# DataZooDE/anofox-forecast

Hardware: AMD Instinct MI355X
Metric: series/sec fit+forecast, AutoETS h=28 on M5-shape batches (higher is better)
Workload: dtype f64

## Files before the change

### anofox-forecast_amd/csrc/det_math.hpp

```cpp
#pragma once
#include <hip/hip_runtime.h>
#include <stdint.h>

namespace anofox {

__device__ __forceinline__ double dm_from_bits(uint64_t u) { return __longlong_as_double((long long)u); }
__device__ __forceinline__ uint64_t dm_bits(double x) { return (uint64_t)__double_as_longlong(x); }

__device__ __forceinline__ double dm_log(double x)
{
    const double ln2_hi = 6.93147180369123816490e-01, ln2_lo = 1.90821492927058770002e-10;
    const double Lg1 = 6.666666666666735130e-01, Lg2 = 3.999999999940941908e-01,
                 Lg3 = 2.857142874366239149e-01, Lg4 = 2.222219843214978396e-01,
                 Lg5 = 1.818357216161805012e-01, Lg6 = 1.531383769920937332e-01,
                 Lg7 = 1.479819860511658591e-01;
    uint64_t u = dm_bits(x);
    uint32_t hx = (uint32_t)(u >> 32);
    int k = 0;
    if (x != x) return x;
    if (hx < 0x00100000u || (hx >> 31)) {
        if ((u << 1) == 0) return -__builtin_huge_val();
        if (hx >> 31) return __builtin_nan("");
        k -= 54;
        x *= 18014398509481984.0;
// ... 145 lines not shown
    const double r2 = r * r;
    const double pa = fma(r, 1.0 / 3.0, -0.5);
    const double pb = fma(r, 0.2, -0.25);
    const double pl = fma(r2, fma(r2, -1.0 / 6.0, pb), pa);
    const double l1p = fma(r2, pl, r);
    const double de = (double)e;
    const double lg = fma(de, ln2_hi, ic.y) + fma(de, ln2_lo, l1p);
    const double t = y * lg;
    const double dn = __builtin_rint(n_per_ln2 * t);
    const double s = fma(-dn, L_lo, fma(-dn, L_hi, t));
    const double s2 = s * s;
    const double qa = fma(s, 1.0 / 6.0, 0.5);
    const double qb = fma(s, 1.0 / 120.0, 1.0 / 24.0);
    const double q = fma(s2, fma(s2, 1.0 / 720.0, qb), qa);
    const double p = fma(s2, q, s);
    const int n = (int)dn;
    const double tv = tab[DM_POW_R64 * (n & 63) + cp.o64];
    const double ev = fma(tv, p, tv);
    return __builtin_ldexp(ev, n >> 6);
}

constexpr int DM_POW_NEAR1_DEG = 11;
constexpr double DM_POW_NEAR1_R = 0x1p-4;
struct DmPowNear1 { double c[DM_POW_NEAR1_DEG + 1]; };
__device__ __forceinline__ void dm_pow_near1_coef(double y, DmPowNear1 &o)
{
    constexpr double inv[DM_POW_NEAR1_DEG + 1] = { 0.0, 1.0, 1.0 / 2.0, 1.0 / 3.0, 1.0 / 4.0, 1.0 / 5.0, 1.0 / 6.0, 1.0 / 7.0,
                                                   1.0 / 8.0, 1.0 / 9.0, 1.0 / 10.0, 1.0 / 11.0 };
    o.c[0] = 1.0;
    o.c[1] = y;
#pragma unroll
    for (int k = 2; k <= DM_POW_NEAR1_DEG; k++) o.c[k] = o.c[k - 1] * ((y - (double)(k - 1)) * inv[k]);
}
__device__ __forceinline__ double dm_pow_near1(double r, const DmPowNear1 &o)
{
    double p = o.c[DM_POW_NEAR1_DEG];
#pragma unroll
    for (int k = DM_POW_NEAR1_DEG - 1; k >= 1; k--) p = fma(p, r, o.c[k]);
    return fma(p, r, 1.0);
}

__device__ __forceinline__ double dm_recip(double d)
{
    const double x0 = __builtin_amdgcn_rcp(d);
    const double e0 = fma(-d, x0, 1.0);
    const double x1 = fma(x0, e0, x0);
    const double e1 = fma(-d, x1, 1.0);
    const double x2 = fma(x1, e1, x1);
    const double e2 = fma(-d, x2, 1.0);
    return fma(e2, x2, x2);
}
__device__ __forceinline__ bool dm_recip_ok(double d) { const double a = fabs(d); return a >= 0x1p-1000 && a <= 0x1p+1000; }

__device__ __forceinline__ double dm_pow_pos(double x, double y) { return dm_exp(y * dm_log(x)); }

}
```

### anofox-forecast_amd/csrc/ets_device.hpp

```cpp
#pragma once
#include <hip/hip_runtime.h>
#include <type_traits>
#include "det_math.hpp"
#include "nm.hpp"

namespace anofox {

enum { C_NONE = 0, C_ADD = 1, C_MUL = 2 };

constexpr double ETS_TOL = 1.0e-10;
constexpr double ETS_HUGEN = 1.0e10;
constexpr double ETS_LN2 = 0.693147180559945309417232121458;
constexpr double PAR_LO = 1.0e-4, PAR_HI = 0.9999, PHI_LO = 0.8, PHI_HI = 0.98;
constexpr int ETS_MERGED_LDS_PERIOD = 16;
constexpr int ETS_LDS_PERIOD = 64;
constexpr int ETS_MAX_PERIOD = 2048;

struct SeriesView {
    const double *y;
    size_t ld;
    int len;
    int wave_len;
    int wave_min_len;
    int rows;
// ... 52 lines not shown
    static constexpr bool CLASSIC = false;
};

struct EtsPar { double alpha, bstar, phi, beta, gamma; DmPowLane pl; DmPowNear1 pc; };
struct EtsState { double l, b, sse, mant; int eacc; int bad; double f; double dlo, dhi, bmin; double rfar; };

template <class Cfg>
__device__ __forceinline__ void ets_unpack(const double (&x)[Cfg::DIM], EtsPar &p)
{
    int k = 0;
    p.alpha = x[k++];
    p.bstar = 0.0;
    double gstar = 0.0;
    p.phi = 1.0;
    if constexpr (Cfg::T != C_NONE) p.bstar = x[k++];
    if constexpr (Cfg::S != C_NONE) gstar = x[k++];
    if constexpr (Cfg::D) p.phi = x[k++];
    p.beta = p.alpha * p.bstar;
    p.gamma = gstar * (1.0 - p.alpha);
}

template <class Cfg, bool NEAR = false>
__device__ __forceinline__ void ets_step(const EtsPar &p, EtsState &st, double y, double &s)
{
    if constexpr (Cfg::ADDITIVE) {
        double phib = 0.0, q = st.l;
        if constexpr (Cfg::T == C_ADD) {
            phib = Cfg::D ? p.phi * st.b : st.b;
            q = st.l + phib;
        }
        double f = q;
        if constexpr (Cfg::S == C_ADD) f = q + s;
        double e = y - f;
        st.sse = fma(e, e, st.sse);
        st.l = fma(p.alpha, e, q);
        st.f = f;
        if constexpr (Cfg::T == C_ADD) st.b = fma(p.beta, e, phib);
        if constexpr (Cfg::S == C_ADD) s = fma(p.gamma, e, s);
    } else {
        double phib = 0.0, q = st.l;
        if constexpr (Cfg::T == C_ADD) {
            phib = Cfg::D ? p.phi * st.b : st.b;
            q = st.l + phib;
        } else if constexpr (Cfg::T == C_MUL) {
            if constexpr (Cfg::D) {
                const double r = st.b - 1.0;
                phib = dm_pow_near1(r, p.pc);
                if constexpr (NEAR) st.rfar = __builtin_fmax(st.rfar, fabs(r));
                else if (!(fabs(r) <= DM_POW_NEAR1_R)) {
                    if (!(st.b >= 0x1p-1000 && st.b <= 0x1p+1000)) st.bad = 1;
                    phib = dm_pow_step(st.b, p.phi, p.pl);
                }
            } else {
                st.bmin = __builtin_fmin(st.bmin, st.b);
                phib = st.b;
            }
            q = st.l * phib;
        }
        double f = q;
        if constexpr (Cfg::S == C_ADD) f = q + s;
        else if constexpr (Cfg::S == C_MUL) f = q * s;
        st.f = f;
        auto recip = [&](const double d) __attribute__((always_inline)) {
            const double ad = fabs(d);
            st.dlo = __builtin_fmin(st.dlo, ad);
            st.dhi = __builtin_fmax(st.dhi, ad);
            return dm_recip(d);
        };
        if constexpr (Cfg::E == C_MUL) {
            static_assert(Cfg::S != C_ADD, "multiplicative error with an additive season is not a valid spec");
            const double rf = recip(f);
            const double eps = (y - f) * rf;
            st.mant = st.mant * fabs(f);
            st.sse = fma(eps, eps, st.sse);
            const double qe = q * eps;
            st.l = fma(p.alpha, qe, q);
            if constexpr (Cfg::T == C_ADD) st.b = fma(p.beta, qe, phib);
            else if constexpr (Cfg::T == C_MUL) st.b = fma(p.beta, phib * eps, phib);
            if constexpr (Cfg::S == C_MUL) s = fma(p.gamma, s * eps, s);
        } else {
            const double e = y - f;
            st.sse = fma(e, e, st.sse);
            if constexpr (Cfg::S == C_MUL && Cfg::T == C_MUL) {
                const double R = recip(f * st.l);
                const double esl = e * (R * q);
                const double es = esl * st.l;
                const double sl = s * st.l;
                st.l = fma(p.alpha, es, q);
                st.b = fma(p.beta, esl, phib);
                s = fma(p.gamma, e * (R * sl), s);
            } else if constexpr (Cfg::S == C_MUL) {
                const double R = recip(f);
                const double es = e * (R * q);
                st.l = fma(p.alpha, es, q);
                if constexpr (Cfg::T == C_ADD) st.b = fma(p.beta, es, phib);
                s = fma(p.gamma, e * (R * s), s);
            } else {
                static_assert(Cfg::T == C_MUL, "general class: a multiplicative component");
                const double rl = recip(st.l);
                st.l = fma(p.alpha, e, q);
                st.b = fma(p.beta, e * rl, phib);
                if constexpr (Cfg::S == C_ADD) s = fma(p.gamma, e, s);
            }
        }
    }
}

template <class Cfg>
__device__ __forceinline__ void ets_renorm(EtsState &st)
{
    if constexpr (Cfg::E == C_MUL) {
        int ex;
        st.mant = frexp(st.mant, &ex);
        st.eacc += ex;
    }
}

template <class Cfg>
__device__ __forceinline__ double ets_objective_value(const EtsState &st, int n)
// ... 10 lines not shown
    if (lik < -1.0e10) lik = -1.0e10;
    return lik;
}

struct EtsInit {
    double l0, b0;
    const double *fig;
    size_t fig_ld;
    int m;
};

struct EtsFinalOut {
    double *yhat; int h; double *sse_out;
    double *fitted; size_t fitted_ld; double *states; size_t states_ld;
    double mean; double *var_out;
};

template <class Cfg, int MS, int K, bool FINAL, class YT = double>
__device__ __forceinline__ void ets_pass(const SeriesView &v, const EtsInit &in,
                                         const double (&cand)[K][Cfg::DIM], double (&fout)[K],
                                         double *ring, const EtsFinalOut *fin)
{
    static_assert((Cfg::S == C_NONE) == (MS == 0), "MS == 0 iff no seasonal component");
    const int lane = threadIdx.x & (NM_BLOCK - 1);
    EtsPar par[K];
    EtsState st[K];
#pragma unroll
    for (int k = 0; k < K; k++) {
        ets_unpack<Cfg>(cand[k], par[k]);
        if constexpr (Cfg::T == C_MUL && Cfg::D) { par[k].pl = dm_pow_lane(); dm_pow_near1_coef(par[k].phi, par[k].pc); }
        st[k].l = in.l0; st[k].b = in.b0; st[k].sse = 0.0; st[k].mant = 1.0; st[k].eacc = 0; st[k].bad = 0;
        st[k].f = 0.0; st[k].dlo = __builtin_huge_val(); st[k].dhi = 0.0; st[k].bmin = __builtin_huge_val(); st[k].rfar = 0.0;

    }
    const double *yp = v.yb;
    const unsigned col_bytes = (unsigned)v.col * (unsigned)sizeof(YT);
    const size_t ld = v.ld;

    const int wave_len = __builtin_amdgcn_readfirstlane(v.wave_len);
    const int wave_min_len = __builtin_amdgcn_readfirstlane(v.wave_min_len);
    const int row_max = __builtin_amdgcn_readfirstlane(v.rows) - 1;
    constexpr int S_WIDE = std::is_same_v<YT, double> ? 1 : (Cfg::ADDITIVE ? ANOFOX_S_COMPACT_MUL_ADD : ANOFOX_S_COMPACT_MUL);
    constexpr int S_FULL = (Cfg::ADDITIVE ? (K == 4 ? (MS > 0 ? ANOFOX_K4_S_SEAS : 16) : 32) : ((Cfg::T == C_MUL && Cfg::D) ? ANOFOX_S_DM : ANOFOX_S_GEN)) * S_WIDE;
    constexpr int S_HBM_CAP = (MS == -2 && !FINAL && !std::is_same_v<YT, double>) ? ANOFOX_S_HBM_RING_COMPACT : 8;
    constexpr int S_TARGET = ((MS == -2 || MS == -4) && K == 1 && S_FULL > S_HBM_CAP) ? S_HBM_CAP : S_FULL;
    constexpr int S = (MS > 0) ? ((S_TARGET / MS > 0 ? S_TARGET / MS : 1) * MS) : S_TARGET;
    typedef std::conditional_t<std::is_same_v<YT, unsigned short>, unsigned, YT> ybuf_t;
    auto widen = [](const ybuf_t x) __attribute__((always_inline)) { return (double)x; };
    ybuf_t cur[S], nxt[S];
    typedef unsigned int u32x2_t __attribute__((ext_vector_type(2)));
    const size_t row_bytes = ld * sizeof(YT);
    const size_t total_bytes = (size_t)(row_max + 1) * row_bytes;
    const int rows_total = row_max + 1;
    auto load_block = [&](ybuf_t (&buf)[S], const int row0) __attribute__((always_inline)) {
        unsigned nrec;
        size_t off;
        if constexpr (Cfg::ADDITIVE) {
            const unsigned rows_left = row0 < rows_total ? (unsigned)(rows_total - row0) : 0u;
            const unsigned long long rem = (unsigned long long)rows_left * (unsigned long long)(unsigned)row_bytes;
            nrec = (unsigned)(rem >> 32) != 0u ? 0xffffffffu : (unsigned)rem;
            off = rows_left ? (size_t)((unsigned long long)(unsigned)row0 * (unsigned long long)(unsigned)row_bytes) : (size_t)0;
        } else {
            const size_t o = (size_t)row0 * row_bytes;
            const size_t rem = o < total_bytes ? total_bytes - o : 0;
            nrec = rem > 0xffffffffull ? 0xffffffffu : (unsigned)rem;
            off = rem ? o : 0;
        }
        const auto rsrc = __builtin_amdgcn_make_buffer_rsrc((void *)((const char *)yp + off), 0, nrec, 0x00020000);
#pragma unroll
        for (int j = 0; j < S; j++) {
            if constexpr (std::is_same_v<YT, double>) {
                const u32x2_t w = __builtin_amdgcn_raw_buffer_load_b64(rsrc, col_bytes, (unsigned)(j * row_bytes), 0);
                buf[j] = __builtin_bit_cast(double, w);
            } else if constexpr (std::is_same_v<YT, float>) {
                const unsigned w = __builtin_amdgcn_raw_buffer_load_b32(rsrc, col_bytes, (unsigned)(j * row_bytes), 0);
                buf[j] = __builtin_bit_cast(float, w);
            } else {
                buf[j] = (unsigned)__builtin_amdgcn_raw_buffer_load_b16(rsrc, col_bytes, (unsigned)(j * row_bytes), 0);
            }
        }
    };
    load_block(cur, 0);
    double var_acc = 0.0;
    auto keep_fit = [&](const int t, const double yv) __attribute__((always_inline)) {
        if constexpr (FINAL) {
            if (fin->fitted && t < v.len) fin->fitted[(size_t)t * fin->fitted_ld] = st[0].f;
            const double dv = yv - fin->mean;
            var_acc += dv * dv;
        }
    };

    if constexpr (MS >= 0) {
        constexpr int MR = MS > 0 ? MS : 1;
        double s[K][MR];
        if constexpr (MS > 0) {
#pragma unroll
            for (int j = 0; j < MS; j++) {
                double f0 = in.fig[(size_t)j * in.fig_ld];
#pragma unroll
                for (int k = 0; k < K; k++) s[k][j] = f0;
            }
        } else {
#pragma unroll
            for (int k = 0; k < K; k++) s[k][0] = 0.0;
        }
        auto run_block = [&](const ybuf_t (&buf)[S], const int base, auto pred_tag) __attribute__((always_inline)) {
            constexpr bool PRED = decltype(pred_tag)::value;
            if constexpr (ANOFOX_DM_RETRY && Cfg::T == C_MUL && Cfg::D && K == 1 && !PRED && !FINAL) {
                const EtsState st0 = st[0];
                double s0[MR];
#pragma unroll
                for (int jj = 0; jj < MR; jj++) s0[jj] = s[0][jj];
                st[0].rfar = 0.0;
#pragma unroll
                for (int j = 0; j < S; j++) {
                    ets_step<Cfg, true>(par[0], st[0], widen(buf[j]), s[0][MS > 0 ? j % MR : 0]);
                    if ((j & 3) == 3 || j == S - 1) ets_renorm<Cfg>(st[0]);
                }
                const bool again = v.len > 0 && (!(st[0].rfar <= DM_POW_NEAR1_R) || st[0].b != st[0].b);
                if (__builtin_amdgcn_ballot_w64(again) == 0ull) return;
                st[0] = st0;
#pragma unroll
                for (int jj = 0; jj < MR; jj++) s[0][jj] = s0[jj];
            }
#pragma unroll
            for (int j = 0; j < S; j++) {
                if (!PRED || base + j < v.len) {
#pragma unroll
                    for (int k = 0; k < K; k++) {
                        ets_step<Cfg>(par[k], st[k], widen(buf[j]), s[k][MS > 0 ? j % MR : 0]);
                        if ((j & 3) == 3 || j == S - 1) ets_renorm<Cfg>(st[k]);
                    }
                    keep_fit(base + j, widen(buf[j]));
                }
            }
        };
        int base = 0;
        constexpr bool TWO = ANOFOX_TWO_BLOCK == 2 || (ANOFOX_TWO_BLOCK == 1 && Cfg::ADDITIVE);
        if constexpr (TWO) {
            for (; base + 2 * S <= wave_min_len; base += 2 * S) {
                load_block(nxt, base + S);
                run_block(cur, base, std::false_type{});
                load_block(cur, base + 2 * S);
                run_block(nxt, base + S, std::false_type{});
            }
        }
        for (; base < wave_len; base += S) {
            load_block(nxt, base + S);
            if (base + S <= wave_min_len) run_block(cur, base, std::false_type{});
            else run_block(cur, base, std::true_type{});
#pragma unroll
            for (int j = 0; j < S; j++) cur[j] = nxt[j];
        }
        if constexpr (FINAL) {
            if constexpr (MS > 0) {
                if (fin->states && v.len > 0) {
#pragma unroll
                    for (int jj = 0; jj < MS; jj++) fin->states[(size_t)(2 + jj) * fin->states_ld] = s[0][jj];
                }
            }
            double pp = par[0].phi, phistar = par[0].phi;
            for (int i = 0; i < fin->h; i++) {
                double f;
                if constexpr (Cfg::T == C_NONE) f = st[0].l;
                else if constexpr (Cfg::T == C_ADD) f = st[0].l + phistar * st[0].b;
                else f = (st[0].b > 0.0) ? st[0].l * dm_pow_pos(st[0].b, phistar) : __builtin_nan("");
                if constexpr (MS > 0) {
                    const int j = (v.len + i) % MS;
                    double sv = s[0][0];
#pragma unroll
                    for (int jj = 1; jj < MS; jj++) sv = (j == jj) ? s[0][jj] : sv;
                    f = (Cfg::S == C_ADD) ? f + sv : f * sv;
                }
                if (v.len > 0) fin->yhat[i] = f;
                pp = pp * par[0].phi;
                phistar = phistar + pp;
            }
        }
    } else {
        constexpr bool LANE_M = MS <= -3;
        static_assert(!LANE_M || K == 1, "per-lane periods: one candidate per lane");
        const int m = LANE_M ? in.m : __builtin_amdgcn_readfirstlane(in.m);
        const int m_max = LANE_M ? __builtin_amdgcn_readfirstlane(wave_max_i32(in.m)) : m;
        for (int j = 0; j < m_max; j++) {
            if (LANE_M && j >= m) continue;
            double f0 = in.fig[(size_t)j * in.fig_ld];
#pragma unroll
            for (int k = 0; k < K; k++) ring[(k * m + j) * NM_BLOCK + lane] = f0;
        }
        int j = 0;
        constexpr bool HBM_RING = (MS == -2 || MS == -4);
        if constexpr (HBM_RING && K == 1) {
            static_assert(2 * S <= ((MS == -2 && !FINAL) ? ETS_LDS_PERIOD : ETS_MERGED_LDS_PERIOD), "the ring prefetch needs periods of at least two blocks");
            double rc[S], rn[S];
            auto ring_load = [&](double (&buf)[S], int j0) __attribute__((always_inline)) {
#pragma unroll
                for (int i = 0; i < S; i++) {
                    buf[i] = ring[(size_t)j0 * NM_BLOCK + lane];
                    j0 = (j0 + 1 == m) ? 0 : j0 + 1;
                }
                return j0;
            };
            int jn = ring_load(rc, 0);
            int base = 0;
            for (; base < wave_len; base += S) {
                load_block(nxt, base + S);
                const int jnn = ring_load(rn, jn);
                const bool full = base + S <= wave_min_len;
#pragma unroll
                for (int i = 0; i < S; i++) {
                    if (full || base + i < v.len) {
                        double sv = rc[i];
                        ets_step<Cfg>(par[0], st[0], widen(cur[i]), sv);
                        if ((i & 3) == 3 || i == S - 1) ets_renorm<Cfg>(st[0]);
                        ring[(size_t)j * NM_BLOCK + lane] = sv;
                        keep_fit(base + i, widen(cur[i]));
                    }
                    j = (j + 1 == m) ? 0 : j + 1;
                }
#pragma unroll
                for (int i = 0; i < S; i++) { cur[i] = nxt[i]; rc[i] = rn[i]; }
                jn = jnn;
            }
        } else {
        auto ring_block = [&](const int base, const bool full) __attribute__((always_inline)) {
#pragma unroll
            for (int i = 0; i < S; i++) {
                if (full || base + i < v.len) {
#pragma unroll
                    for (int k = 0; k < K; k++) {
                        double sv = ring[(k * m + j) * NM_BLOCK + lane];
                        ets_step<Cfg>(par[k], st[k], widen(cur[i]), sv);
                        if ((i & 3) == 3 || i == S - 1) ets_renorm<Cfg>(st[k]);
                        ring[(k * m + j) * NM_BLOCK + lane] = sv;
                    }
                    keep_fit(base + i, widen(cur[i]));
                }
                j = (j + 1 == m) ? 0 : j + 1;
            }
        };
        int base = 0;
        for (; base < wave_len; base += S) {
            load_block(nxt, base + S);
            ring_block(base, base + S <= wave_min_len);
#pragma unroll
            for (int i = 0; i < S; i++) cur[i] = nxt[i];
        }
        }
        if constexpr (FINAL) {
            if (fin->states && v.len > 0)
                for (int jj = 0; jj < m; jj++) fin->states[(size_t)(2 + jj) * fin->states_ld] = ring[(0 * m + jj) * NM_BLOCK + lane];
            double pp = par[0].phi, phistar = par[0].phi;
            for (int i = 0; i < fin->h; i++) {
                double f;
                if constexpr (Cfg::T == C_NONE) f = st[0].l;
                else if constexpr (Cfg::T == C_ADD) f = st[0].l + phistar * st[0].b;
                else f = (st[0].b > 0.0) ? st[0].l * dm_pow_pos(st[0].b, phistar) : __builtin_nan("");
                const int jj = (v.len + i) % m;
                double sv = ring[(0 * m + jj) * NM_BLOCK + lane];
                f = (Cfg::S == C_ADD) ? f + sv : f * sv;
                if (v.len > 0) fin->yhat[i] = f;
                pp = pp * par[0].phi;
                phistar = phistar + pp;
            }
        }
    }
#pragma unroll
    for (int k = 0; k < K; k++) {
        ets_renorm<Cfg>(st[k]);
        fout[k] = ets_objective_value<Cfg>(st[k], v.len);
    }
    if constexpr (FINAL) {
        if (fin->sse_out && v.len > 0) *fin->sse_out = st[0].sse;
        if (fin->var_out) *fin->var_out = var_acc;
        if (fin->states && v.len > 0) { fin->states[0] = st[0].l; fin->states[fin->states_ld] = Cfg::T != C_NONE ? st[0].b : __builtin_nan(""); }
    }
}

template <class Cfg, int MS, int CPL, class YT = double>
struct EtsModel {
    static constexpr int DIM = Cfg::DIM;
    SeriesView v;
    EtsInit in;
    double *ring;
    __device__ void bounds(double (&lo)[DIM], double (&hi)[DIM], double (&x0)[DIM]) const
    {
        int k = 0;
        lo[k] = PAR_LO; hi[k] = PAR_HI; x0[k] = 0.3; k++;
        if constexpr (Cfg::T != C_NONE) { lo[k] = PAR_LO; hi[k] = PAR_HI; x0[k] = 0.1; k++; }
        if constexpr (Cfg::S != C_NONE) { lo[k] = PAR_LO; hi[k] = PAR_HI; x0[k] = 0.1; k++; }
        if constexpr (Cfg::D) { lo[k] = PHI_LO; hi[k] = PHI_HI; x0[k] = 0.9; k++; }
    }
    __device__ double eval1(const double (&x)[DIM]) const
    {
        double c1[1][DIM], f1[1];
#pragma unroll
        for (int i = 0; i < DIM; i++) c1[0][i] = x[i];
        ets_pass<Cfg, MS, 1, false, YT>(v, in, c1, f1, ring, nullptr);
        return f1[0];
// ... 21 lines not shown
```

### anofox-forecast_amd/csrc/ets_fit_kernel.hpp

```cpp
#pragma once
#include "ets_device.hpp"
#include "classic_device.hpp"
#include "kernels.hpp"

#ifndef ANOFOX_ROUND_WAVES
#define ANOFOX_ROUND_WAVES 2
#endif
namespace anofox {

#ifndef ANOFOX_PARK_CLASS
#define ANOFOX_PARK_CLASS 0
#endif
#ifndef ANOFOX_PARK_WAVES
#define ANOFOX_PARK_WAVES 4
#endif
#ifndef ANOFOX_DM_WPB
#define ANOFOX_DM_WPB 1
#endif
#ifndef ANOFOX_SETPRIO
#define ANOFOX_SETPRIO 0
#endif
#ifndef ANOFOX_ROUND_WAVES_COMPACT
#define ANOFOX_ROUND_WAVES_COMPACT ANOFOX_ROUND_WAVES
#endif
#ifndef ANOFOX_SEQ_WAVES_COMPACT
#define ANOFOX_SEQ_WAVES_COMPACT 0
#endif
template <class Cfg, class YT = double> struct RoundTraits {
    static constexpr bool DAMPED_MUL = !Cfg::CLASSIC && Cfg::T == C_MUL && Cfg::D;
    static constexpr bool PARK = !Cfg::CLASSIC && (ANOFOX_PARK_CLASS >= 3 || (ANOFOX_PARK_CLASS == 2 && !Cfg::ADDITIVE) || (ANOFOX_PARK_CLASS == 1 && DAMPED_MUL));
    static constexpr int WAVES = PARK ? ANOFOX_PARK_WAVES : (std::is_same_v<YT, double> ? ANOFOX_ROUND_WAVES : ANOFOX_ROUND_WAVES_COMPACT);
    static constexpr int WPB = DAMPED_MUL ? ANOFOX_DM_WPB : 1;
};

template <class Cfg, int MS, class YT = double, bool CLASSIC = Cfg::CLASSIC> struct RoundModelOf { using type = EtsModel<Cfg, MS, 1, YT>; };
template <class Cfg, int MS, class YT> struct RoundModelOf<Cfg, MS, YT, true> { using type = ClassicRoundModel<Cfg::KIND, MS>; };

template <class Cfg, int MS, int SPEC, bool K4 = false, class YT = double>
__device__ __forceinline__ void ets_round_body(const FitArgs &a, const int vblock, const int vgrid, const int wave, double *const lds_all)
{
    constexpr int D = Cfg::DIM;
    constexpr bool PARK = RoundTraits<Cfg>::PARK;
    if constexpr (ANOFOX_SETPRIO >= 1 && RoundTraits<Cfg>::DAMPED_MUL) __builtin_amdgcn_s_setprio(3);
    else if constexpr (ANOFOX_SETPRIO >= 2 && !Cfg::CLASSIC && !Cfg::ADDITIVE) __builtin_amdgcn_s_setprio(ANOFOX_SETPRIO == 2 ? 1 : 2);
    if (a.wave_prio == 3) __builtin_amdgcn_s_setprio(3);
    else if (a.wave_prio == 2) __builtin_amdgcn_s_setprio(2);
    else if (a.wave_prio == 1) __builtin_amdgcn_s_setprio(1);
    if constexpr (Cfg::T == C_MUL && Cfg::D) dm_pow_tab_init();
    const int lane = threadIdx.x & (NM_BLOCK - 1);
    const int lds_per_wave = (PARK ? 0 : nm_lds_doubles<D>()) + ((MS == -1 || MS == -3) ? a.m * NM_BLOCK : 0);
    double *const lds = lds_all + (size_t)wave * (size_t)lds_per_wave;
    double *const nmst = PARK ? a.nm_scratch + (size_t)vblock * (size_t)nm_lds_doubles<D>() : lds;
    double *const lds_ring = PARK ? lds : lds + nm_lds_doubles<D>();
    const unsigned long long trace_t0 = a.wave_trace ? __builtin_amdgcn_s_memrealtime() : 0ull;
    const int n_act = a.n_active ? *a.n_active : a.n_series;
    int mode = SPEC;
    if constexpr (SPEC == 3) mode = n_act > a.spec_below ? 0 : ((a.spec2_below > 0 && n_act <= a.spec2_below && n_act <= vgrid) ? 2 : 1);
    else if (a.spec_below >= 0) {
        const int owner = n_act > a.spec_below ? 0 : (n_act > a.spec2_below ? 1 : 2);
        if (owner != SPEC) return;
    }
    const int LPP = mode == 0 ? 1 : (mode == 1 ? NM_K : NM_BLOCK);
    const int PPB = NM_BLOCK / LPP;
    if (vblock * PPB >= n_act) return;
    const int p = vblock * PPB + lane / LPP;
    const bool valid = p < n_act;
    const int s = valid ? (a.series_of ? a.series_of[p] : p) : 0;
    const int len = valid ? a.len[s] : 0;

    const int m = a.m_col ? (MS <= -3 ? a.m_col[s] : __builtin_amdgcn_readfirstlane(a.m_col[s])) : a.m;
    const int n_param = a.n_param - ((Cfg::S != C_NONE && a.m_col) ? a.m - m : 0);
    bool active = valid;
    if (!a.first_round && a.series_of == nullptr && valid && a.st.done[s]) active = false;
    if (a.first_round) {
        int st = FIT_OK;
        if constexpr (Cfg::CLASSIC) {
            const int min_len = Cfg::KIND == CK_HW ? 2 * m : (Cfg::KIND == CK_SEASONAL_ES ? m : a.min_len);
            if (len <= 0 || (a.mask != nullptr && valid && a.mask[s] != a.want)) st = FIT_SKIPPED;
            else if (len < min_len) st = FIT_SHORT;
        } else {
            const uint32_t fl = valid ? a.flags[s] : 0u;
            if (len <= 0) st = FIT_SKIPPED;
            else if (Cfg::S != C_NONE && len < 2 * m) st = FIT_SHORT;
            else if (len < n_param + 2) st = FIT_SHORT;
            else if (a.need_positive && !(fl & SF_POSITIVE)) st = FIT_NONPOSITIVE;
            else if (a.skip_constant && (fl & SF_CONSTANT)) st = FIT_SKIPPED;
        }
        active = valid && st == FIT_OK;
        if (valid) {
            a.status[s] = st;
            if (!active) { a.st.done[s] = 1; a.st.passes[s] = 0; a.st.evals[s] = 0; a.st.iters[s] = 0; }
        }
    }

    SeriesView v;
    const bool gathered = a.gathered != 0 && n_act <= a.gather_cap;
    v.col = valid ? (gathered ? p : s) : 0;
    v.yb = gathered ? a.y_round : a.y;
    v.y = v.yb + v.col;
    v.ld = gathered ? a.ld_round : a.ld;
    v.len = active ? len : 0;
    v.wave_len = wave_max_i32(v.len);
    v.wave_min_len = wave_min_i32(active ? len : 0x7fffffff);
    v.rows = a.t_rows;
    if (v.wave_len == 0) return;

    typename RoundModelOf<Cfg, MS, YT>::type mdl;
    mdl.v = v;
    mdl.in.l0 = (active && !Cfg::CLASSIC) ? a.l0[s] : 0.0;
    mdl.in.b0 = (active && !Cfg::CLASSIC && Cfg::T != C_NONE) ? a.b0[s] : 0.0;
    mdl.in.fig = a.fig ? a.fig + s : nullptr;
    mdl.in.fig_ld = a.fig_ld;
    mdl.in.m = m;
    mdl.ring = (MS == -2 || MS == -4) ? a.ring_scratch + (size_t)vblock * (size_t)a.m * NM_BLOCK : lds_ring;

    NmRun r;
// ... 217 lines not shown
```

### anofox-forecast_amd/csrc/ets_group_kernel.hpp

```cpp
#pragma once
#include "fit_units.hpp"

namespace anofox {

template <int ID, int MSG> constexpr int group_member_ms()
{
    if constexpr (SpecOf<ID>::s == 0) return 0;
    else if constexpr (MSG == 12 && !SpecOf<ID>::Cfg::ADDITIVE) return -1;
    else return MSG;
}
template <int ID, int MSG> constexpr bool group_member_k4() { return SpecOf<ID>::Cfg::ADDITIVE && (group_member_ms<ID, MSG>() == 0 || group_member_ms<ID, MSG>() == 7); }

template <class YT, int... IDS> struct GroupTraits {
    static constexpr bool OK = ((RoundTraits<typename SpecOf<IDS>::Cfg, YT>::WAVES == RoundTraits<typename SpecOf<0>::Cfg, YT>::WAVES &&
                                 RoundTraits<typename SpecOf<IDS>::Cfg>::WPB == 1 && !RoundTraits<typename SpecOf<IDS>::Cfg>::PARK) && ...);
};

template <class YT> constexpr int group_waves = RoundTraits<typename SpecOf<0>::Cfg, YT>::WAVES;

template <int ID, int MSG, class YT>
__device__ __forceinline__ void ets_group_slot(const FitArgs &a, const int k4, const int vblock, const int vgrid, double *const lds)
{
    using Cfg = typename SpecOf<ID>::Cfg;
    constexpr int MS = group_member_ms<ID, MSG>();
    if constexpr (SpecOf<ID>::s != 0 && MSG == 0) return;
    else {
        if constexpr (group_member_k4<ID, MSG>())
            if (k4) { ets_round_body<Cfg, MS, 3, true, YT>(a, vblock, vgrid, 0, lds); return; }
        ets_round_body<Cfg, MS, 3, false, YT>(a, vblock, vgrid, 0, lds);
    }
}

template <int MSG, class YT, int... IDS>
__global__ __launch_bounds__(NM_BLOCK, group_waves<YT>) void ets_group_round_kernel(const FitArgs *__restrict__ tab, const GroupRoundArgs g)
{
    extern __shared__ double lds_all[];
    const int b = (int)blockIdx.x;
    int k = 0;
    while (k + 1 < g.n_slots && b >= g.start[k + 1]) k++;
    const FitArgs &a = *(const FitArgs *)((const __attribute__((address_space(4))) FitArgs *)tab + k);
    const int vblock = b - g.start[k], vgrid = g.start[k + 1] - g.start[k], id = g.spec[k], k4 = g.k4[k];
    (void)((id == IDS && (ets_group_slot<IDS, MSG, YT>(a, k4, vblock, vgrid, lds_all), true)) || ...);
}

template <int MSG, class YT, int... IDS>
void ets_group_round_launch(const FitArgs *tab, const GroupRoundArgs &g, int m, hipStream_t stream)
{
    const int blocks = g.start[g.n_slots];
    if (blocks <= 0) return;
    size_t lds_doubles = 0;
    ((lds_doubles = std::max(lds_doubles, (size_t)nm_lds_doubles<SpecOf<IDS>::Cfg::DIM>() +
                                              (group_member_ms<IDS, MSG>() == -1 ? (size_t)m * NM_BLOCK : 0))), ...);
    const size_t lds_bytes = sizeof(double) * lds_doubles;
    if (lds_bytes > 48 * 1024)
        anofox_check_attr(hipFuncSetAttribute((const void *)ets_group_round_kernel<MSG, YT, IDS...>, hipFuncAttributeMaxDynamicSharedMemorySize, (int)lds_bytes));
    hipLaunchKernelGGL((ets_group_round_kernel<MSG, YT, IDS...>), dim3(blocks), dim3(NM_BLOCK), lds_bytes, stream, tab, g);
}

template <int MSG, int... IDS> GroupLaunchFn group_launcher_of_yt(int yt)
{
    if constexpr (!GroupTraits<double, IDS...>::OK || !GroupTraits<float, IDS...>::OK) return nullptr;
    else {
        if (yt == YT_U16) {
            if constexpr (ets_u16_variant(MSG) && GroupTraits<unsigned short, IDS...>::OK) return &ets_group_round_launch<MSG, unsigned short, IDS...>;
            else return nullptr;
        }
        if (yt == YT_F32) return &ets_group_round_launch<MSG, float, IDS...>;
        return &ets_group_round_launch<MSG, double, IDS...>;
    }
}
template <int... IDS> GroupLaunchFn group_launcher_of(int m, int yt)
{
    if (m <= 1) return group_launcher_of_yt<0, IDS...>(yt);
    if (m == 7) return group_launcher_of_yt<7, IDS...>(yt);
    constexpr bool ring12 = ((SpecOf<IDS>::s != 0 && SpecOf<IDS>::Cfg::ADDITIVE) || ...);
    if (m == 12 && ring12) return group_launcher_of_yt<12, IDS...>(yt);
    if (m > ETS_LDS_PERIOD) return group_launcher_of_yt<-2, IDS...>(yt);
    return group_launcher_of_yt<-1, IDS...>(yt);
}

}
```

### anofox-forecast_amd/csrc/kernels.hip

```cpp
#include "classic_device.hpp"
#include "fit_units.hpp"
#include "kernels.hpp"

namespace anofox {

__global__ __launch_bounds__(NM_BLOCK) void select_kernel(const SelectArgs a)
{
    const int s = blockIdx.x * NM_BLOCK + threadIdx.x;
    if (s >= a.n_series) return;
    if (a.len[s] <= 0) { a.fallback_mask[s] = 0u; return; }
    int best = -1;
    double best_aicc = __builtin_huge_val();
    int passes = 0, evals = 0;
    for (int k = 0; k < a.n_slots; k++) {
        passes += a.passes_slots[(size_t)k * a.ld + s];
        evals += a.evals_slots[(size_t)k * a.ld + s];
        if (a.status_slots[(size_t)k * a.ld + s] != FIT_OK) continue;
        double v = a.aicc[(size_t)k * a.ld + s];
        if (v < best_aicc) { best_aicc = v; best = k; }
    }
    a.passes_total[s] = passes;
    a.evals_total[s] = evals;
    if (best < 0) {
        a.status[s] = -1;
// ... 219 lines not shown
    bool keep = false;
    if (idx < n_prev) {
        s = series_prev ? series_prev[idx] : idx;
        keep = done[s] == 0;
    }
    const unsigned long long bal = __ballot(keep);
    const int cnt = __popcll(bal);
    if (cnt == 0) return;
    int base = 0;
    if (lane == 0) base = atomicAdd(n_next_ptr, cnt);
    base = __shfl(base, 0);
    const int before = __popcll(bal & ((1ull << lane) - 1ull));
    if (keep) series_next[base + before] = s;
}

void launch_compact(const int32_t *series_prev, const int32_t *n_prev, int n_series, const int32_t *done,
                    int32_t *series_next, int32_t *n_next, hipStream_t stream, int32_t *n_clear)
{
    if (!n_clear) anofox_check_attr(hipMemsetAsync(n_next, 0, sizeof(int32_t), stream));
    const int grid = (n_series + NM_BLOCK - 1) / NM_BLOCK;
    hipLaunchKernelGGL(compact_kernel, dim3(grid), dim3(NM_BLOCK), 0, stream, series_prev, n_prev, n_series, done, series_next, n_next, n_clear);
}

constexpr int GATHER_TB = 32;
template <class E>
__global__ __launch_bounds__(NM_BLOCK) void gather_columns_kernel(const E *y, size_t ld, const int32_t *series_of,
                                                                  const int32_t *n_active, int t_max, E *out, size_t ld_out, int cap)
{
    const int n_act = *n_active;
    if ((int)blockIdx.x * NM_BLOCK >= n_act || n_act > cap) return;
    const int p = blockIdx.x * NM_BLOCK + threadIdx.x;
    const int s = series_of[p < n_act ? p : n_act - 1];
    const int t0 = blockIdx.y * GATHER_TB;
    const int t1 = t0 + GATHER_TB < t_max ? t0 + GATHER_TB : t_max;
    for (int t = t0; t < t1; t++) out[(size_t)t * ld_out + p] = y[(size_t)t * ld + s];
}

void launch_gather_columns(const void *y, size_t ld, const int32_t *series_of, const int32_t *n_active, int n_series,
                           int t_max, void *out, size_t ld_out, hipStream_t stream, int cap, int elem_bytes)
{
    if (n_series <= 0 || t_max <= 0) return;
    const int n_cols = std::min(n_series, cap);
    if (n_cols <= 0) return;
    dim3 grid((n_cols + NM_BLOCK - 1) / NM_BLOCK, (t_max + GATHER_TB - 1) / GATHER_TB);
    if (elem_bytes == 8)
        hipLaunchKernelGGL(gather_columns_kernel<double>, grid, dim3(NM_BLOCK), 0, stream, (const double *)y, ld, series_of, n_active, t_max, (double *)out, ld_out, cap);
    else if (elem_bytes == 4)
        hipLaunchKernelGGL(gather_columns_kernel<float>, grid, dim3(NM_BLOCK), 0, stream, (const float *)y, ld, series_of, n_active, t_max, (float *)out, ld_out, cap);
    else
        hipLaunchKernelGGL(gather_columns_kernel<unsigned short>, grid, dim3(NM_BLOCK), 0, stream, (const unsigned short *)y, ld, series_of, n_active, t_max, (unsigned short *)out, ld_out, cap);
}

constexpr int GROUP_COMPACT_BLOCKS = 256, GROUP_GATHER_COL_BLOCKS = 128, GROUP_GATHER_ROW_BLOCKS = 8;
__global__ __launch_bounds__(NM_BLOCK) void group_compact_kernel(const GroupCompactArgs g)
{
    const int k = blockIdx.y;
    if (g.n_clear[k] && blockIdx.x == 0 && threadIdx.x == 0) *g.n_clear[k] = 0;
    const int n_prev = g.n_prev[k] ? *g.n_prev[k] : g.n_series;
    const int32_t *prev = g.prev[k], *done = g.done[k];
    const int lane = threadIdx.x;
    for (int base0 = (int)blockIdx.x * NM_BLOCK; base0 < n_prev; base0 += (int)gridDim.x * NM_BLOCK) {
        const int idx = base0 + lane;
        int s = 0;
        bool keep = false;
        if (idx < n_prev) {
            s = prev ? prev[idx] : idx;
            keep = done[s] == 0;
        }
        const unsigned long long bal = __ballot(keep);
        const int cnt = __popcll(bal);
        if (cnt == 0) continue;
        int base = 0;
        if (lane == 0) base = atomicAdd(g.n_next[k], cnt);
        base = __shfl(base, 0);
        const int before = __popcll(bal & ((1ull << lane) - 1ull));
        if (keep) g.next[k][base + before] = s;
    }
}

void launch_group_compact(const GroupCompactArgs &g, hipStream_t stream)
{
    if (g.n_slots <= 0 || g.n_series <= 0) return;
    const int grid = std::min((g.n_series + NM_BLOCK - 1) / NM_BLOCK, GROUP_COMPACT_BLOCKS);
    hipLaunchKernelGGL(group_compact_kernel, dim3(grid, g.n_slots), dim3(NM_BLOCK), 0, stream, g);
}

struct GroupZeroArgs { int32_t *p[GROUP_MAX_SLOTS]; };
__global__ void group_zero3_kernel(const int n, const GroupZeroArgs z)
{
    const int i = threadIdx.x;
    if (i < 3 * n) z.p[i / 3][i % 3] = 0;
}

void launch_group_zero3(int n, int32_t *const *zero, hipStream_t stream)
{
    if (n <= 0) return;
    GroupZeroArgs z{};
    for (int k = 0; k < n && k < GROUP_MAX_SLOTS; k++) z.p[k] = zero[k];
    hipLaunchKernelGGL(group_zero3_kernel, dim3(1), dim3(64), 0, stream, std::min(n, GROUP_MAX_SLOTS), z);
}

template <class E>
__global__ __launch_bounds__(NM_BLOCK) void group_gather_kernel(const GroupGatherArgs g)
{
    const int k = blockIdx.z;
    const int n_act = *g.n_active[k];
    if (n_act > g.cap[k]) return;
    const E *y = (const E *)g.y;
    E *out = (E *)g.out[k];
    const size_t ld_out = g.ld_out[k];
    const int32_t *series_of = g.series_of[k];
    for (int p0 = (int)blockIdx.x * NM_BLOCK; p0 < n_act; p0 += (int)gridDim.x * NM_BLOCK) {
        const int p = p0 + (int)threadIdx.x;
        const int s = series_of[p < n_act ? p : n_act - 1];
        for (int t0 = (int)blockIdx.y * GATHER_TB; t0 < g.t_max; t0 += (int)gridDim.y * GATHER_TB) {
            const int t1 = t0 + GATHER_TB < g.t_max ? t0 + GATHER_TB : g.t_max;
            for (int t = t0; t < t1; t++) out[(size_t)t * ld_out + p] = y[(size_t)t * g.ld + s];
        }
    }
}

void launch_group_gather(const GroupGatherArgs &g, int n_cols_max, hipStream_t stream)
{
    if (g.n_slots <= 0 || g.t_max <= 0 || n_cols_max <= 0) return;
    dim3 grid(std::min((n_cols_max + NM_BLOCK - 1) / NM_BLOCK, GROUP_GATHER_COL_BLOCKS),
              std::min((g.t_max + GATHER_TB - 1) / GATHER_TB, GROUP_GATHER_ROW_BLOCKS), g.n_slots);
    if (g.elem_bytes == 8) hipLaunchKernelGGL(group_gather_kernel<double>, grid, dim3(NM_BLOCK), 0, stream, g);
    else if (g.elem_bytes == 4) hipLaunchKernelGGL(group_gather_kernel<float>, grid, dim3(NM_BLOCK), 0, stream, g);
    else hipLaunchKernelGGL(group_gather_kernel<unsigned short>, grid, dim3(NM_BLOCK), 0, stream, g);
}

__global__ __launch_bounds__(NM_BLOCK) void compact_block_kernel(const double *y, size_t ld, const int32_t *len, int n_series, int t_rows, float *out32,
                                                                 unsigned short *out16, unsigned int *misfit)
{
    const int s = blockIdx.x * NM_BLOCK + threadIdx.x;
    const int t0 = blockIdx.y * GATHER_TB;
    const int t1 = t0 + GATHER_TB < t_rows ? t0 + GATHER_TB : t_rows;
    const int L = s < n_series ? len[s] : 0;
    unsigned bad32 = 0, bad16 = 0;
    if ((size_t)s < ld) {
        for (int t = t0; t < t1; t++) {
            const double v = y[(size_t)t * ld + s];
            const float f = (float)v;
            const unsigned short u = (v >= 0.0 && v <= 65535.0) ? (unsigned short)v : (unsigned short)0;
            out32[(size_t)t * ld + s] = f;
            if (out16) out16[(size_t)t * ld + s] = u;
            if (t < L) {
                bad32 += (__double_as_longlong((double)f) == __double_as_longlong(v)) ? 0u : 1u;
                bad16 += (__double_as_longlong((double)u) == __double_as_longlong(v)) ? 0u : 1u;
            }
        }
    }
#pragma unroll
    for (int o = 32; o >= 1; o >>= 1) { bad32 += __shfl_xor(bad32, o); bad16 += __shfl_xor(bad16, o); }
    if (threadIdx.x == 0) {
        if (bad32) atomicAdd(misfit, bad32);
        if (bad16) atomicAdd(misfit + 1, bad16);
    }
}

void launch_compact_block(const double *y, size_t ld, const int32_t *len, int n_series, int t_rows, float *out32, unsigned short *out16,
                          unsigned int *misfit, hipStream_t stream)
{
    if (ld == 0 || t_rows <= 0) return;
    dim3 grid((unsigned)((ld + NM_BLOCK - 1) / NM_BLOCK), (unsigned)((t_rows + GATHER_TB - 1) / GATHER_TB));
    hipLaunchKernelGGL(compact_block_kernel, grid, dim3(NM_BLOCK), 0, stream, y, ld, len, n_series, t_rows, out32, out16, misfit);
}

constexpr int DETECT_THREADS = 256;
template <bool USE_LDS>
__global__ __launch_bounds__(DETECT_THREADS) void detect_period_kernel(const double *y, size_t ld, const int32_t *len, int n_series, int t_rows,
                                                                       double *scratch, int32_t *period, double *best_acf_out)
{
    extern __shared__ double detect_lds[];
    __shared__ double sh_mean, sh_var;
    const int tid = threadIdx.x;
    double *c = USE_LDS ? detect_lds : scratch + (size_t)blockIdx.x * ((size_t)t_rows + (size_t)t_rows / 2 + 2);
    double *acf = c + t_rows;
    for (int s = blockIdx.x; s < n_series; s += gridDim.x) {
        const int n = len[s];
        int best = 0;
        double best_acf = 0.0;
// ... 104 lines not shown
```

Baseline: 80380.

## Refill input buffer in place and use fused abs min/max asm

Adds inline-asm v_min_f64/v_max_f64 helpers that fold the absolute-value modifier into the min/max used to track bounds. For non-additive configs with narrow input types, the double-buffered block loads (cur and nxt arrays) are replaced by an in-place refill. Each slot is widened and then immediately reloaded with the next block's row, which removes the nxt buffer and the copy loop. This is meant to reduce VGPR pressure and instruction count in the ETS fit loops. The trade-off is that the loads are interleaved with the compute, and the inline asm may limit compiler scheduling and skip its NaN-handling semantics.

```diff
diff --git a/anofox-forecast_amd/csrc/det_math.hpp b/anofox-forecast_amd/csrc/det_math.hpp
--- a/anofox-forecast_amd/csrc/det_math.hpp
+++ b/anofox-forecast_amd/csrc/det_math.hpp
@@ -221,6 +221,25 @@
 }
 __device__ __forceinline__ bool dm_recip_ok(double d) { const double a = fabs(d); return a >= 0x1p-1000 && a <= 0x1p+1000; }
 
+__device__ __forceinline__ double dm_track_min(double t, double x)
+{
+    double r;
+    asm("v_min_f64 %0, %1, %2" : "=v"(r) : "v"(t), "v"(x));
+    return r;
+}
+__device__ __forceinline__ double dm_track_min_abs(double t, double x)
+{
+    double r;
+    asm("v_min_f64 %0, %1, |%2|" : "=v"(r) : "v"(t), "v"(x));
+    return r;
+}
+__device__ __forceinline__ double dm_track_max_abs(double t, double x)
+{
+    double r;
+    asm("v_max_f64 %0, %1, |%2|" : "=v"(r) : "v"(t), "v"(x));
+    return r;
+}
+
 __device__ __forceinline__ double dm_pow_pos(double x, double y) { return dm_exp(y * dm_log(x)); }
 
 }
diff --git a/anofox-forecast_amd/csrc/ets_device.hpp b/anofox-forecast_amd/csrc/ets_device.hpp
--- a/anofox-forecast_amd/csrc/ets_device.hpp
+++ b/anofox-forecast_amd/csrc/ets_device.hpp
@@ -128,7 +128,7 @@
                     phib = dm_pow_step(st.b, p.phi, p.pl);
                 }
             } else {
-                st.bmin = __builtin_fmin(st.bmin, st.b);
+                st.bmin = dm_track_min(st.bmin, st.b);
                 phib = st.b;
             }
             q = st.l * phib;
@@ -138,9 +138,8 @@
         else if constexpr (Cfg::S == C_MUL) f = q * s;
         st.f = f;
         auto recip = [&](const double d) __attribute__((always_inline)) {
-            const double ad = fabs(d);
-            st.dlo = __builtin_fmin(st.dlo, ad);
-            st.dhi = __builtin_fmax(st.dhi, ad);
+            st.dlo = dm_track_min_abs(st.dlo, d);
+            st.dhi = dm_track_max_abs(st.dhi, d);
             return dm_recip(d);
         };
         if constexpr (Cfg::E == C_MUL) {
@@ -257,7 +256,7 @@
     const size_t row_bytes = ld * sizeof(YT);
     const size_t total_bytes = (size_t)(row_max + 1) * row_bytes;
     const int rows_total = row_max + 1;
-    auto load_block = [&](ybuf_t (&buf)[S], const int row0) __attribute__((always_inline)) {
+    auto block_rsrc = [&](const int row0) __attribute__((always_inline)) {
         unsigned nrec;
         size_t off;
         if constexpr (Cfg::ADDITIVE) {
@@ -271,19 +270,32 @@
             nrec = rem > 0xffffffffull ? 0xffffffffu : (unsigned)rem;
             off = rem ? o : 0;
         }
-        const auto rsrc = __builtin_amdgcn_make_buffer_rsrc((void *)((const char *)yp + off), 0, nrec, 0x00020000);
-#pragma unroll
-        for (int j = 0; j < S; j++) {
-            if constexpr (std::is_same_v<YT, double>) {
-                const u32x2_t w = __builtin_amdgcn_raw_buffer_load_b64(rsrc, col_bytes, (unsigned)(j * row_bytes), 0);
-                buf[j] = __builtin_bit_cast(double, w);
-            } else if constexpr (std::is_same_v<YT, float>) {
-                const unsigned w = __builtin_amdgcn_raw_buffer_load_b32(rsrc, col_bytes, (unsigned)(j * row_bytes), 0);
-                buf[j] = __builtin_bit_cast(float, w);
-            } else {
-                buf[j] = (unsigned)__builtin_amdgcn_raw_buffer_load_b16(rsrc, col_bytes, (unsigned)(j * row_bytes), 0);
-            }
-        }
+        return __builtin_amdgcn_make_buffer_rsrc((void *)((const char *)yp + off), 0, nrec, 0x00020000);
+    };
+    typedef decltype(block_rsrc(0)) rsrc_t;
+    auto load_row = [&](const rsrc_t rsrc, const int j) __attribute__((always_inline)) -> ybuf_t {
+        if constexpr (std::is_same_v<YT, double>) {
+            const u32x2_t w = __builtin_amdgcn_raw_buffer_load_b64(rsrc, col_bytes, (unsigned)(j * row_bytes), 0);
+            return __builtin_bit_cast(double, w);
+        } else if constexpr (std::is_same_v<YT, float>) {
+            const unsigned w = __builtin_amdgcn_raw_buffer_load_b32(rsrc, col_bytes, (unsigned)(j * row_bytes), 0);
+            return __builtin_bit_cast(float, w);
+        } else {
+            return (unsigned)__builtin_amdgcn_raw_buffer_load_b16(rsrc, col_bytes, (unsigned)(j * row_bytes), 0);
+        }
+    };
+    auto load_block = [&](ybuf_t (&buf)[S], const int row0) __attribute__((always_inline)) {
+        const rsrc_t rsrc = block_rsrc(row0);
+#pragma unroll
+        for (int j = 0; j < S; j++) buf[j] = load_row(rsrc, j);
+    };
+    constexpr bool REFILL = !Cfg::ADDITIVE && !std::is_same_v<YT, double> && ANOFOX_TWO_BLOCK != 2 && !ANOFOX_DM_RETRY;
+    constexpr bool PIN_WIDEN = REFILL && Cfg::T == C_MUL && Cfg::D;
+    auto take_row = [&](ybuf_t &slot, const rsrc_t next, const int j) __attribute__((always_inline)) {
+        double yv = widen(slot);
+        if constexpr (PIN_WIDEN) asm volatile("" : "+v"(yv));
+        slot = load_row(next, j);
+        return yv;
     };
     load_block(cur, 0);
     double var_acc = 0.0;
@@ -337,6 +349,22 @@
                         if ((j & 3) == 3 || j == S - 1) ets_renorm<Cfg>(st[k]);
                     }
                     keep_fit(base + j, widen(buf[j]));
+                }
+            }
+        };
+        auto refill_block = [&](const int base, auto pred_tag) __attribute__((always_inline)) {
+            constexpr bool PRED = decltype(pred_tag)::value;
+            const rsrc_t next = block_rsrc(base + S);
+#pragma unroll
+            for (int j = 0; j < S; j++) {
+                const double yv = take_row(cur[j], next, j);
+                if (!PRED || base + j < v.len) {
+#pragma unroll
+                    for (int k = 0; k < K; k++) {
+                        ets_step<Cfg>(par[k], st[k], yv, s[k][MS > 0 ? j % MR : 0]);
+                        if ((j & 3) == 3 || j == S - 1) ets_renorm<Cfg>(st[k]);
+                    }
+                    keep_fit(base + j, yv);
                 }
             }
         };
@@ -350,12 +378,17 @@
                 run_block(nxt, base + S, std::false_type{});
             }
         }
-        for (; base < wave_len; base += S) {
-            load_block(nxt, base + S);
-            if (base + S <= wave_min_len) run_block(cur, base, std::false_type{});
-            else run_block(cur, base, std::true_type{});
-#pragma unroll
-            for (int j = 0; j < S; j++) cur[j] = nxt[j];
+        if constexpr (REFILL) {
+            for (; base + S <= wave_min_len; base += S) refill_block(base, std::false_type{});
+            for (; base < wave_len; base += S) refill_block(base, std::true_type{});
+        } else {
+            for (; base < wave_len; base += S) {
+                load_block(nxt, base + S);
+                if (base + S <= wave_min_len) run_block(cur, base, std::false_type{});
+                else run_block(cur, base, std::true_type{});
+#pragma unroll
+                for (int j = 0; j < S; j++) cur[j] = nxt[j];
+            }
         }
         if constexpr (FINAL) {
             if constexpr (MS > 0) {
@@ -428,28 +461,36 @@
                 jn = jnn;
             }
         } else {
+        constexpr bool RING_REFILL = REFILL && !HBM_RING;
         auto ring_block = [&](const int base, const bool full) __attribute__((always_inline)) {
+            const rsrc_t next = block_rsrc(base + S);
 #pragma unroll
             for (int i = 0; i < S; i++) {
+                const double yv = RING_REFILL ? take_row(cur[i], next, i) : widen(cur[i]);
                 if (full || base + i < v.len) {
 #pragma unroll
                     for (int k = 0; k < K; k++) {
                         double sv = ring[(k * m + j) * NM_BLOCK + lane];
-                        ets_step<Cfg>(par[k], st[k], widen(cur[i]), sv);
+                        ets_step<Cfg>(par[k], st[k], yv, sv);
                         if ((i & 3) == 3 || i == S - 1) ets_renorm<Cfg>(st[k]);
                         ring[(k * m + j) * NM_BLOCK + lane] = sv;
                     }
-                    keep_fit(base + i, widen(cur[i]));
+                    keep_fit(base + i, yv);
                 }
                 j = (j + 1 == m) ? 0 : j + 1;
             }
         };
         int base = 0;
-        for (; base < wave_len; base += S) {
-            load_block(nxt, base + S);
-            ring_block(base, base + S <= wave_min_len);
-#pragma unroll
-            for (int i = 0; i < S; i++) cur[i] = nxt[i];
+        if constexpr (RING_REFILL) {
+            for (; base + S <= wave_min_len; base += S) ring_block(base, true);
+            for (; base < wave_len; base += S) ring_block(base, false);
+        } else {
+            for (; base < wave_len; base += S) {
+                load_block(nxt, base + S);
+                ring_block(base, base + S <= wave_min_len);
+#pragma unroll
+                for (int i = 0; i < S; i++) cur[i] = nxt[i];
+            }
         }
         }
         if constexpr (FINAL) {
```

After: 81880, median of 6. 1.9% higher.

## Pack live workgroups to the front of grouped round, compact and gather grids

Applied to the files above, without the earlier changes.

The grouped kernels now map block indices only onto live work. Each slot contributes as many blocks as its active series count needs, so the blocks that would exit immediately are all trailing and dispatched contiguously at the end. The same live-block mapping is applied to the compact and gather kernels by flattening their multi-dimensional grids into one dimension. The damped-multiplicative power table init is also deferred until after the early exit, so dead blocks skip it. In exchange, every block performs a serial scan over the slots and reads device-side active counts, and the grid size still covers the worst case.

```diff
diff --git a/anofox-forecast_amd/csrc/ets_fit_kernel.hpp b/anofox-forecast_amd/csrc/ets_fit_kernel.hpp
--- a/anofox-forecast_amd/csrc/ets_fit_kernel.hpp
+++ b/anofox-forecast_amd/csrc/ets_fit_kernel.hpp
@@ -2,6 +2,7 @@
 #include "ets_device.hpp"
 #include "classic_device.hpp"
 #include "kernels.hpp"
+#include "ets_group_mapping.hpp"
 
 #ifndef ANOFOX_ROUND_WAVES
 #define ANOFOX_ROUND_WAVES 2
@@ -46,7 +47,6 @@
     if (a.wave_prio == 3) __builtin_amdgcn_s_setprio(3);
     else if (a.wave_prio == 2) __builtin_amdgcn_s_setprio(2);
     else if (a.wave_prio == 1) __builtin_amdgcn_s_setprio(1);
-    if constexpr (Cfg::T == C_MUL && Cfg::D) dm_pow_tab_init();
     const int lane = threadIdx.x & (NM_BLOCK - 1);
     const int lds_per_wave = (PARK ? 0 : nm_lds_doubles<D>()) + ((MS == -1 || MS == -3) ? a.m * NM_BLOCK : 0);
     double *const lds = lds_all + (size_t)wave * (size_t)lds_per_wave;
@@ -55,13 +55,15 @@
     const unsigned long long trace_t0 = a.wave_trace ? __builtin_amdgcn_s_memrealtime() : 0ull;
     const int n_act = a.n_active ? *a.n_active : a.n_series;
     int mode = SPEC;
-    if constexpr (SPEC == 3) mode = n_act > a.spec_below ? 0 : ((a.spec2_below > 0 && n_act <= a.spec2_below && n_act <= vgrid) ? 2 : 1);
+    if constexpr (SPEC == 3) mode = round_auto_mode(n_act, a.spec_below, a.spec2_below, vgrid);
     else if (a.spec_below >= 0) {
         const int owner = n_act > a.spec_below ? 0 : (n_act > a.spec2_below ? 1 : 2);
         if (owner != SPEC) return;
     }
     const int LPP = mode == 0 ? 1 : (mode == 1 ? NM_K : NM_BLOCK);
     const int PPB = NM_BLOCK / LPP;
+    if ((vblock - wave) * PPB >= n_act) return;
+    if constexpr (Cfg::T == C_MUL && Cfg::D) dm_pow_tab_init();
     if (vblock * PPB >= n_act) return;
     const int p = vblock * PPB + lane / LPP;
     const bool valid = p < n_act;
diff --git a/anofox-forecast_amd/csrc/ets_group_kernel.hpp b/anofox-forecast_amd/csrc/ets_group_kernel.hpp
--- a/anofox-forecast_amd/csrc/ets_group_kernel.hpp
+++ b/anofox-forecast_amd/csrc/ets_group_kernel.hpp
@@ -35,11 +35,15 @@
 __global__ __launch_bounds__(NM_BLOCK, group_waves<YT>) void ets_group_round_kernel(const FitArgs *__restrict__ tab, const GroupRoundArgs g)
 {
     extern __shared__ double lds_all[];
-    const int b = (int)blockIdx.x;
-    int k = 0;
-    while (k + 1 < g.n_slots && b >= g.start[k + 1]) k++;
-    const FitArgs &a = *(const FitArgs *)((const __attribute__((address_space(4))) FitArgs *)tab + k);
-    const int vblock = b - g.start[k], vgrid = g.start[k + 1] - g.start[k], id = g.spec[k], k4 = g.k4[k];
+    const auto *const ctab = (const __attribute__((address_space(4))) FitArgs *)tab;
+    const GroupLiveBlock w = group_live_block((int)blockIdx.x, g.n_slots, [&](const int j) {
+        const FitArgs &s = *(const FitArgs *)(ctab + j);
+        return group_slot_live(s.n_active ? *s.n_active : s.n_series, s.spec_below, s.spec2_below, g.start[j + 1] - g.start[j], NM_BLOCK, NM_K);
+    });
+    if (w.slot < 0) return;
+    const int k = w.slot;
+    const FitArgs &a = *(const FitArgs *)(ctab + k);
+    const int vblock = w.vblock, vgrid = g.start[k + 1] - g.start[k], id = g.spec[k], k4 = g.k4[k];
     (void)((id == IDS && (ets_group_slot<IDS, MSG, YT>(a, k4, vblock, vgrid, lds_all), true)) || ...);
 }
 
diff --git a/anofox-forecast_amd/csrc/ets_group_mapping.hpp b/anofox-forecast_amd/csrc/ets_group_mapping.hpp
--- /dev/null
+++ b/anofox-forecast_amd/csrc/ets_group_mapping.hpp
@@ -0,0 +1,42 @@
+#pragma once
+
+#if defined(__HIPCC__) || defined(__CUDACC__)
+#define ANOFOX_HD __host__ __device__
+#else
+#define ANOFOX_HD
+#endif
+
+namespace anofox {
+
+ANOFOX_HD inline int round_auto_mode(const int n_act, const int spec_below, const int spec2_below, const int vgrid)
+{
+    return n_act > spec_below ? 0 : ((spec2_below > 0 && n_act <= spec2_below && n_act <= vgrid) ? 2 : 1);
+}
+
+ANOFOX_HD inline int live_workgroups(const int n, const int per, const int cap)
+{
+    if (n <= 0 || cap <= 0) return 0;
+    const int need = (int)(((long long)n + per - 1) / per);
+    return need < cap ? need : cap;
+}
+
+ANOFOX_HD inline int group_slot_live(const int n_act, const int spec_below, const int spec2_below, const int cap, const int nm_block, const int nm_k)
+{
+    const int mode = round_auto_mode(n_act, spec_below, spec2_below, cap);
+    return live_workgroups(n_act, mode == 0 ? nm_block : (mode == 1 ? nm_block / nm_k : 1), cap);
+}
+
+struct GroupLiveBlock { int slot, vblock; };
+
+template <class LiveOf> ANOFOX_HD inline GroupLiveBlock group_live_block(const int b, const int n_slots, LiveOf live_of)
+{
+    int base = 0;
+    for (int k = 0; k < n_slots; k++) {
+        const int live = live_of(k);
+        if (b - base < live) return GroupLiveBlock{k, b - base};
+        base += live;
+    }
+    return GroupLiveBlock{-1, 0};
+}
+
+}
diff --git a/anofox-forecast_amd/csrc/kernels.hip b/anofox-forecast_amd/csrc/kernels.hip
--- a/anofox-forecast_amd/csrc/kernels.hip
+++ b/anofox-forecast_amd/csrc/kernels.hip
@@ -295,14 +295,18 @@
 }
 
 constexpr int GROUP_COMPACT_BLOCKS = 256, GROUP_GATHER_COL_BLOCKS = 128, GROUP_GATHER_ROW_BLOCKS = 8;
-__global__ __launch_bounds__(NM_BLOCK) void group_compact_kernel(const GroupCompactArgs g)
-{
-    const int k = blockIdx.y;
-    if (g.n_clear[k] && blockIdx.x == 0 && threadIdx.x == 0) *g.n_clear[k] = 0;
+__global__ __launch_bounds__(NM_BLOCK) void group_compact_kernel(const GroupCompactArgs g, const int cap)
+{
+    if ((int)blockIdx.x < g.n_slots && g.n_clear[blockIdx.x] && threadIdx.x == 0) *g.n_clear[blockIdx.x] = 0;
+    const GroupLiveBlock w = group_live_block((int)blockIdx.x, g.n_slots, [&](const int j) {
+        return live_workgroups(g.n_prev[j] ? *g.n_prev[j] : g.n_series, NM_BLOCK, cap);
+    });
+    if (w.slot < 0) return;
+    const int k = w.slot;
     const int n_prev = g.n_prev[k] ? *g.n_prev[k] : g.n_series;
     const int32_t *prev = g.prev[k], *done = g.done[k];
     const int lane = threadIdx.x;
-    for (int base0 = (int)blockIdx.x * NM_BLOCK; base0 < n_prev; base0 += (int)gridDim.x * NM_BLOCK) {
+    for (int base0 = w.vblock * NM_BLOCK; base0 < n_prev; base0 += cap * NM_BLOCK) {
         const int idx = base0 + lane;
         int s = 0;
         bool keep = false;
@@ -324,8 +328,8 @@
 void launch_group_compact(const GroupCompactArgs &g, hipStream_t stream)
 {
     if (g.n_slots <= 0 || g.n_series <= 0) return;
-    const int grid = std::min((g.n_series + NM_BLOCK - 1) / NM_BLOCK, GROUP_COMPACT_BLOCKS);
-    hipLaunchKernelGGL(group_compact_kernel, dim3(grid, g.n_slots), dim3(NM_BLOCK), 0, stream, g);
+    const int cap = std::min((g.n_series + NM_BLOCK - 1) / NM_BLOCK, GROUP_COMPACT_BLOCKS);
+    hipLaunchKernelGGL(group_compact_kernel, dim3(cap * g.n_slots), dim3(NM_BLOCK), 0, stream, g, cap);
 }
 
 struct GroupZeroArgs { int32_t *p[GROUP_MAX_SLOTS]; };
@@ -344,19 +348,25 @@
 }
 
 template <class E>
-__global__ __launch_bounds__(NM_BLOCK) void group_gather_kernel(const GroupGatherArgs g)
-{
-    const int k = blockIdx.z;
+__global__ __launch_bounds__(NM_BLOCK) void group_gather_kernel(const GroupGatherArgs g, const int col_blocks, const int row_blocks)
+{
+    const auto live_cols = [&](const int j) {
+        const int n = *g.n_active[j];
+        return n > g.cap[j] ? 0 : live_workgroups(n, NM_BLOCK, col_blocks);
+    };
+    const GroupLiveBlock w = group_live_block((int)blockIdx.x, g.n_slots, [&](const int j) { return live_cols(j) * row_blocks; });
+    if (w.slot < 0) return;
+    const int k = w.slot;
     const int n_act = *g.n_active[k];
-    if (n_act > g.cap[k]) return;
+    const int lc = live_cols(k), bx = w.vblock % lc, by = w.vblock / lc;
     const E *y = (const E *)g.y;
     E *out = (E *)g.out[k];
     const size_t ld_out = g.ld_out[k];
     const int32_t *series_of = g.series_of[k];
-    for (int p0 = (int)blockIdx.x * NM_BLOCK; p0 < n_act; p0 += (int)gridDim.x * NM_BLOCK) {
+    for (int p0 = bx * NM_BLOCK; p0 < n_act; p0 += col_blocks * NM_BLOCK) {
         const int p = p0 + (int)threadIdx.x;
         const int s = series_of[p < n_act ? p : n_act - 1];
-        for (int t0 = (int)blockIdx.y * GATHER_TB; t0 < g.t_max; t0 += (int)gridDim.y * GATHER_TB) {
+        for (int t0 = by * GATHER_TB; t0 < g.t_max; t0 += row_blocks * GATHER_TB) {
             const int t1 = t0 + GATHER_TB < g.t_max ? t0 + GATHER_TB : g.t_max;
             for (int t = t0; t < t1; t++) out[(size_t)t * ld_out + p] = y[(size_t)t * g.ld + s];
         }
@@ -366,11 +376,12 @@
 void launch_group_gather(const GroupGatherArgs &g, int n_cols_max, hipStream_t stream)
 {
     if (g.n_slots <= 0 || g.t_max <= 0 || n_cols_max <= 0) return;
-    dim3 grid(std::min((n_cols_max + NM_BLOCK - 1) / NM_BLOCK, GROUP_GATHER_COL_BLOCKS),
-              std::min((g.t_max + GATHER_TB - 1) / GATHER_TB, GROUP_GATHER_ROW_BLOCKS), g.n_slots);
-    if (g.elem_bytes == 8) hipLaunchKernelGGL(group_gather_kernel<double>, grid, dim3(NM_BLOCK), 0, stream, g);
-    else if (g.elem_bytes == 4) hipLaunchKernelGGL(group_gather_kernel<float>, grid, dim3(NM_BLOCK), 0, stream, g);
-    else hipLaunchKernelGGL(group_gather_kernel<unsigned short>, grid, dim3(NM_BLOCK), 0, stream, g);
+    const int col_blocks = std::min((n_cols_max + NM_BLOCK - 1) / NM_BLOCK, GROUP_GATHER_COL_BLOCKS);
+    const int row_blocks = std::min((g.t_max + GATHER_TB - 1) / GATHER_TB, GROUP_GATHER_ROW_BLOCKS);
+    const dim3 grid(col_blocks * row_blocks * g.n_slots);
+    if (g.elem_bytes == 8) hipLaunchKernelGGL(group_gather_kernel<double>, grid, dim3(NM_BLOCK), 0, stream, g, col_blocks, row_blocks);
+    else if (g.elem_bytes == 4) hipLaunchKernelGGL(group_gather_kernel<float>, grid, dim3(NM_BLOCK), 0, stream, g, col_blocks, row_blocks);
+    else hipLaunchKernelGGL(group_gather_kernel<unsigned short>, grid, dim3(NM_BLOCK), 0, stream, g, col_blocks, row_blocks);
 }
 
 __global__ __launch_bounds__(NM_BLOCK) void compact_block_kernel(const double *y, size_t ld, const int32_t *len, int n_series, int t_rows, float *out32,
```

After: 78680 before, 79790 after, median of 6. 1.4% higher.
